# Joao-M-Silva/padel_analytics

Measured on NVIDIA H100. Metric: frames/sec through trackers.runner (all 4 trackers), higher is better.
Workload: dtype f16 storage, f32 accumulate

## Files before the change

padel_analytics_b200/csrc/conv_common.cuh:

```cuda
#pragma once
#include "internal.h"
#include "ptx.cuh"

namespace pb {

__device__ __forceinline__ void bias_act16(const uint32_t (&r)[16], const float* __restrict__ sbias, int act,
                                           float (&v)[16], const __half* __restrict__ res_first = nullptr) {
#pragma unroll
  for (int q = 0; q < 4; ++q) {
    const float4 b = *reinterpret_cast<const float4*>(sbias + 4 * q);
    v[4 * q + 0] = __uint_as_float(r[4 * q + 0]) + b.x;
    v[4 * q + 1] = __uint_as_float(r[4 * q + 1]) + b.y;
    v[4 * q + 2] = __uint_as_float(r[4 * q + 2]) + b.z;
    v[4 * q + 3] = __uint_as_float(r[4 * q + 3]) + b.w;
  }
  if (res_first != nullptr) {
#pragma unroll
    for (int j = 0; j < 16; ++j) v[j] += __half2float(res_first[j]);
  }
  if (act == PB_ACT_SILU) {
#pragma unroll
    for (int i = 0; i < 16; ++i) v[i] = __fdividef(v[i], 1.f + __expf(-v[i]));
  } else if (act == PB_ACT_RELU) {
#pragma unroll
// ... 101 lines not shown
  } else if (kp.out_mode == PB_OUT_F32_NCHW) {
    float* ob = reinterpret_cast<float*>(kp.out);
    const size_t plane = (size_t)kp.Ho * kp.Wo;
    const size_t base = (size_t)px.n * kp.cout_store * plane + (size_t)px.oh * kp.Wo + px.ow;
#pragma unroll
    for (int j = 0; j < 16; ++j)
      if (ch0 + j < kp.cout_store) ob[base + (size_t)(ch0 + j) * plane] = v[j];
  }
}

__device__ __forceinline__ bool epilogue_fast_ok(const ConvKParams& kp) {
  if ((kp.dbg_flags & 2) != 0 && kp.out2_mode == PB_OUT2_NONE) return false;
  if (kp.head_n != 0 || (kp.res != nullptr && ((kp.res_C | kp.res_coff) & 7) != 0)) return false;
  if ((reinterpret_cast<uintptr_t>(kp.out) & 31) != 0) return false;
  if (kp.out_mode == PB_OUT_F16_NHWC || kp.out_mode == PB_OUT_F16_NHWC_UP2)
    return ((kp.out_C | kp.out_coff) & 15) == 0 && (kp.cout_store & 15) == 0;
  if (kp.out_mode == PB_OUT_F32_NHWC) return ((kp.out_C | kp.out_coff) & 7) == 0;
  return false;
}

__device__ __forceinline__ void silu4(float& a, float& b, float& c, float& d) {
  constexpr float kNegLog2e = -1.4426950408889634f;
  const float da = 1.f + ex2_approx(fminf(a * kNegLog2e, 30.f));
  const float db = 1.f + ex2_approx(fminf(b * kNegLog2e, 30.f));
  const float dc = 1.f + ex2_approx(fminf(c * kNegLog2e, 30.f));
  const float dd = 1.f + ex2_approx(fminf(d * kNegLog2e, 30.f));
  const float pab = da * db, pcd = dc * dd;
  const float r = rcp_approx(pab * pcd);
  const float rab = pcd * r, rcd = pab * r;
  a *= db * rab;
  b *= da * rab;
  c *= dd * rcd;
  d *= dc * rcd;
}

struct EpiOut {
  int mode;
  size_t dx, dy;
  int mode2;
  size_t dx2, dy2;
  bool pool_writer;
};

__device__ __forceinline__ void epi_add_res16(const uint4 (&rv)[2], float (&v)[16]) {
#pragma unroll
  for (int g = 0; g < 2; ++g) {
    const __half2* h2 = reinterpret_cast<const __half2*>(&rv[g]);
#pragma unroll
    for (int j = 0; j < 4; ++j) {
      const float2 f = __half22float2(h2[j]);
      v[8 * g + 2 * j] = __fadd_rn(v[8 * g + 2 * j], f.x);
      v[8 * g + 2 * j + 1] = __fadd_rn(v[8 * g + 2 * j + 1], f.y);
    }
  }
}

__device__ __forceinline__ void epi_compute16(int act, int has_res, bool plain_silu, uint32_t (&r)[16],
                                              const float* __restrict__ sbias, const uint4 (&rv)[2], float (&v)[16]) {
#pragma unroll
  for (int q = 0; q < 4; ++q) {
    const float4 b = *reinterpret_cast<const float4*>(sbias + 4 * q);
    v[4 * q + 0] = __uint_as_float(r[4 * q + 0]) + b.x;
    v[4 * q + 1] = __uint_as_float(r[4 * q + 1]) + b.y;
    v[4 * q + 2] = __uint_as_float(r[4 * q + 2]) + b.z;
    v[4 * q + 3] = __uint_as_float(r[4 * q + 3]) + b.w;
  }
// ... 262 lines not shown
```

padel_analytics_b200/csrc/conv_halo.cu:

```cuda
#include <cstdlib>
#include <mutex>
#include <vector>

#include "conv_halo_kernel.cuh"

namespace pb {


static void halo_finish_config(ConvPlan* plan) {
  const ConvKParams& kp = plan->kp;
  plan->smem_bytes = (size_t)kp.a_stages * kp.a_bytes + (size_t)kp.b_stages * kp.b_bytes + sizeof(HaloSmemTail) + 1024;
  plan->threads = kConvThreads;
  plan->grid = kp.total_tiles < num_sms() ? kp.total_tiles : num_sms();
}

int conv_stem_setup(const pb_conv_desc* d, ConvPlan* plan, EncodeTiledFn encode) {
  PB_CHECK(d->ksize == 3 && d->stride == 2 && d->C == 4 && d->cin == 16 && d->c_in_off == 0,
           "conv(stem): needs ksize 3, stride 2, C = 4, cin = 16");
  PB_CHECK(d->cout_pad <= 128, "conv(stem): cout_pad %d > 128", d->cout_pad);
  ConvKParams& kp = plan->kp;
  const int BN = d->cout_pad;
  const int acc_cols = (BN + 31) / 32 * 32;
  int S = 4;
  while (S > 1 && S * acc_cols > 2 * kConvAccRegs) S >>= 1;
  kp.KB = 16;
  kp.kblocks = 1;
  kp.taps = 3;
  kp.hs_S = S;
  kp.hs_P = 8 * S;
  kp.hs_G = 3;
  kp.hs_ntaps = 3;
  kp.hs_sbo_rows = 3 * 8 * S;
  kp.hs_x0 = 0;
  kp.hs_y0 = 0;
  for (int r = 0; r < 3; ++r) kp.hs_tap_off[r] = r * 8 * S;
  for (int r = 0; r < 3; ++r) kp.hs_tap_desc[r] = (kp.hs_tap_off[r] * 32) >> 4;
  kp.BN = BN;
  kp.n_ntiles = 1;
  kp.halo_bytes = 16u * 3u * (uint32_t)(8 * S) * 32u;
  kp.hs_a_row_bytes = 32u;
  const uint32_t pairs = (uint32_t)(8 * S) + 1;
  const uint32_t pitch = pairs * 16u;
  static const int raw = [] {
    const char* e = getenv("PADEL_B200_STEM_RAW");
    return e ? atoi(e) : 1;
  }();
  if (raw) {
    kp.halo_bytes = 17u * 2u * pitch;
    kp.hs_a_row_bytes = 16u;
    kp.hs_sbo_rows = (int)(2u * pitch / 16u);
    for (int r = 0; r < 3; ++r) kp.hs_tap_desc[r] = (int)(((uint32_t)r * pitch) >> 4);
  }
  kp.a_bytes = (kp.halo_bytes + 1023u) & ~1023u;
  kp.b_tx_bytes = 3u * (uint32_t)BN * 32u;
  kp.b_bytes = (kp.b_tx_bytes + 1023u) & ~1023u;
  kp.a_stages = 4;
  kp.b_stages = 1;
  kp.b_resident = 1;
  kp.tiles_w = (kp.Wo + 8 * S - 1) / (8 * S);
  kp.tiles_h = (kp.Ho + 15) / 16;
  kp.tiles_n = kp.N;
  kp.total_tiles = kp.tiles_w * kp.tiles_h * kp.tiles_n;
  halo_finish_config(plan);
  plan->variant = 1;
  {
    const cuuint64_t Wp = (cuuint64_t)d->W + 2, Hp = (cuuint64_t)d->H + 2;
    cuuint64_t dims[5] = {16, (cuuint64_t)d->W / 2, 3, (cuuint64_t)d->H / 2, (cuuint64_t)d->N};
    cuuint64_t strides[4] = {16, Wp * 8, 2 * Wp * 8, Hp * Wp * 8};
    cuuint32_t box[5] = {16, (cuuint32_t)(8 * S), 3, 16, 1};
    cuuint32_t estr[5] = {1, 1, 1, 1, 1};
    CUtensorMapSwizzle swz = CU_TENSOR_MAP_SWIZZLE_32B;
    if (raw) {
      dims[0] = 8, dims[1] = Wp / 2, dims[2] = 2, dims[3] = Hp / 2;
      strides[0] = 16, strides[1] = Wp * 8, strides[2] = 2 * Wp * 8;
      box[0] = 8, box[1] = pairs, box[2] = 2, box[3] = 17;
      swz = CU_TENSOR_MAP_SWIZZLE_NONE;
    }
    CUresult r = encode(&plan->tmap_a, CU_TENSOR_MAP_DATA_TYPE_FLOAT16, 5, const_cast<void*>(d->in), dims, strides,
                        box, estr, CU_TENSOR_MAP_INTERLEAVE_NONE, swz, CU_TENSOR_MAP_L2_PROMOTION_L2_128B,
                        CU_TENSOR_MAP_FLOAT_OOB_FILL_NONE);
    PB_CHECK(r == CUDA_SUCCESS, "conv(stem): cuTensorMapEncodeTiled(A, overlapping rows) failed with %d", (int)r);
  }
  {
    cuuint64_t dims[3] = {16, (cuuint64_t)d->cout_pad, 3};
    cuuint64_t strides[2] = {32, (cuuint64_t)d->cout_pad * 32};
    cuuint32_t box[3] = {16, (cuuint32_t)BN, 3};
    cuuint32_t estr[3] = {1, 1, 1};
    CUresult r = encode(&plan->tmap_w, CU_TENSOR_MAP_DATA_TYPE_FLOAT16, 3, const_cast<void*>(d->weight), dims,
                        strides, box, estr, CU_TENSOR_MAP_INTERLEAVE_NONE, CU_TENSOR_MAP_SWIZZLE_32B,
                        CU_TENSOR_MAP_L2_PROMOTION_L2_256B, CU_TENSOR_MAP_FLOAT_OOB_FILL_NONE);
    PB_CHECK(r == CUDA_SUCCESS, "conv(stem): cuTensorMapEncodeTiled(W) failed with %d", (int)r);
  }
  return 0;
}

int conv_halo_setup(const pb_conv_desc* d, ConvPlan* plan, EncodeTiledFn encode) {
  if (d->ksize != 3 || d->stride != 1 || d->cout_pad > 256) return -1;
  ConvKParams& kp = plan->kp;
  const int BN = d->cout_pad;
  const uint32_t row_bytes = (uint32_t)kp.KB * 2u;
  const int acc_cols = (BN + 31) / 32 * 32;
  const size_t budget = 196 * 1024;
  const uint32_t tap_bytes = (uint32_t)BN * row_bytes;
  const uint32_t res_box = (9u * tap_bytes + 1023u) & ~1023u;
  const size_t res_total = (size_t)kp.kblocks * res_box;
  bool resident = false;
  {
    const char* er = getenv("PADEL_B200_CONV_BRES");
    resident = (!er || atoi(er) != 0) && kp.kblocks <= kHaloMaxB && res_total <= 120 * 1024;
  }
  int bestS = 0, best_cols = 0, G = 1;
  for (int pass = resident ? 0 : 1; pass < 2 && bestS == 0; ++pass) {
    resident = resident && pass == 0;
    for (int S = 4; S >= 1; S >>= 1) {
      if (S * acc_cols > 2 * kConvAccRegs) continue;
      const uint32_t halo = 18u * (uint32_t)(8 * S + 2) * row_bytes;
      const uint32_t a_alloc = (halo + 1023u) & ~1023u;
      int g_fit = 0;
      if (resident) {
        if ((size_t)2 * a_alloc + res_total <= budget) g_fit = 9;
      } else {
        for (int g = 9; g >= 1; g = (g == 9 ? 3 : (g == 3 ? 1 : 0))) {
          const uint32_t ba = ((uint32_t)g * tap_bytes + 1023u) & ~1023u;
          const int min_b = g == 9 ? 2 : (g == 3 ? 3 : 4);
          if ((size_t)2 * a_alloc + (size_t)min_b * ba <= budget) {
            g_fit = g;
            break;
          }
        }
      }
      if (!g_fit) continue;
      const int cols = (d->W + 8 * S - 1) / (8 * S) * 8 * S;
      if (bestS == 0 || (!resident && cols < best_cols)) {
        bestS = S;
        best_cols = cols;
// ... 17 lines not shown
      kp.hs_tap_off[r * 3 + q] = r * P + q;
      kp.hs_tap_desc[r * 3 + q] = (int)(((uint32_t)(r * P + q) * row_bytes) >> 4);
    }
  kp.BN = BN;
  kp.n_ntiles = 1;
  kp.halo_bytes = 18u * (uint32_t)P * row_bytes;
  kp.hs_a_row_bytes = row_bytes;
  kp.a_bytes = (kp.halo_bytes + 1023u) & ~1023u;
  kp.b_tx_bytes = (uint32_t)G * tap_bytes;
  kp.b_bytes = b_alloc;
  kp.a_stages = 2;
  if (resident) {
    kp.b_stages = kp.kblocks;
    int as = (int)((budget - res_total) / kp.a_bytes);
    if (as > kHaloMaxA) as = kHaloMaxA;
    if (as > 2 * kp.kblocks + 1) as = 2 * kp.kblocks + 1;
    kp.a_stages = as < 2 ? 2 : as;
  } else {
    size_t rest = budget - (size_t)2 * kp.a_bytes;
    if (kp.kblocks > 2 && rest > (size_t)kp.a_bytes + 4 * (size_t)b_alloc) {
      kp.a_stages = 3;
      rest -= kp.a_bytes;
    }
    int bs = (int)(rest / b_alloc);
    if (bs > kHaloMaxB) bs = kHaloMaxB;
    if (bs > 9 * kp.kblocks / G * 2) bs = 9 * kp.kblocks / G * 2;
    if (bs < 2) bs = 2;
    kp.b_stages = bs;
  }
  kp.tiles_w = (kp.Wo + 8 * S - 1) / (8 * S);
  kp.tiles_h = (kp.Ho + 15) / 16;
  kp.tiles_n = kp.N;
  kp.total_tiles = kp.tiles_w * kp.tiles_h * kp.tiles_n;
  halo_finish_config(plan);
  plan->variant = 1;

  const CUtensorMapSwizzle swz = kp.KB == 64   ? CU_TENSOR_MAP_SWIZZLE_128B
                                 : kp.KB == 32 ? CU_TENSOR_MAP_SWIZZLE_64B
                                               : CU_TENSOR_MAP_SWIZZLE_32B;
  {
    const cuuint64_t C = (cuuint64_t)d->C, W = (cuuint64_t)d->W, H = (cuuint64_t)d->H;
    cuuint64_t dims[5] = {C, W, 1, H, (cuuint64_t)d->N};
    cuuint64_t strides[4] = {C * 2, W * C * 2, W * C * 2, H * W * C * 2};
    cuuint32_t box[5] = {(cuuint32_t)kp.KB, (cuuint32_t)P, 1, 18, 1};
    cuuint32_t estr[5] = {1, 1, 1, 1, 1};
    CUresult r = encode(&plan->tmap_a, CU_TENSOR_MAP_DATA_TYPE_FLOAT16, 5, const_cast<void*>(d->in), dims, strides,
                        box, estr, CU_TENSOR_MAP_INTERLEAVE_NONE, swz, CU_TENSOR_MAP_L2_PROMOTION_L2_128B,
                        CU_TENSOR_MAP_FLOAT_OOB_FILL_NONE);
    PB_CHECK(r == CUDA_SUCCESS, "conv(halo): cuTensorMapEncodeTiled(A) failed with %d", (int)r);
  }
  {
    cuuint64_t dims[3] = {(cuuint64_t)d->cin, (cuuint64_t)d->cout_pad, 9};
    cuuint64_t strides[2] = {(cuuint64_t)d->cin * 2, (cuuint64_t)d->cin * d->cout_pad * 2};
    cuuint32_t box[3] = {(cuuint32_t)kp.KB, (cuuint32_t)BN, (cuuint32_t)G};
    cuuint32_t estr[3] = {1, 1, 1};
    CUresult r = encode(&plan->tmap_w, CU_TENSOR_MAP_DATA_TYPE_FLOAT16, 3, const_cast<void*>(d->weight), dims,
                        strides, box, estr, CU_TENSOR_MAP_INTERLEAVE_NONE, swz, CU_TENSOR_MAP_L2_PROMOTION_L2_256B,
                        CU_TENSOR_MAP_FLOAT_OOB_FILL_NONE);
    PB_CHECK(r == CUDA_SUCCESS, "conv(halo): cuTensorMapEncodeTiled(W) failed with %d", (int)r);
  }
  return 0;
}

int conv_halo_1x1_setup(const pb_conv_desc* d, ConvPlan* plan, EncodeTiledFn encode) {
  static const int enabled = [] {
    const char* e = getenv("PADEL_B200_CONV_HALO1");
    return e ? atoi(e) : 1;
  }();
  if (!enabled || d->ksize != 1 || d->stride != 1 || d->cout_pad > 256 || d->head_n != 0) return -1;
  if (enabled == 1 && d->cin > 32) return -1;
  if (d->out_mode != PB_OUT_F16_NHWC && d->out_mode != PB_OUT_F16_NHWC_UP2) return -1;
  ConvKParams& kp = plan->kp;
  const int BN = d->cout_pad;
  const uint32_t row_bytes = (uint32_t)kp.KB * 2u;
  const int acc_cols = (BN + 31) / 32 * 32;
  const size_t budget = 196 * 1024;
  const uint32_t tap_bytes = (uint32_t)BN * row_bytes;
  const uint32_t res_box = (tap_bytes + 1023u) & ~1023u;
  const size_t res_total = (size_t)kp.kblocks * res_box;
  if (kp.kblocks > kHaloMaxB || res_total > 120 * 1024) return -1;
  int S = 0;
  for (int s = 4; s >= 1; s >>= 1) {
    if (s * acc_cols > 2 * kConvAccRegs) continue;
    const uint32_t a_alloc = (16u * (uint32_t)(8 * s) * row_bytes + 1023u) & ~1023u;
    if ((size_t)2 * a_alloc + res_total > budget) continue;
    if (s > 1 && d->W <= 8 * (s / 2)) continue;
    S = s;
    break;
  }
  if (S == 0) return -1;
  const int P = 8 * S;
  kp.b_resident = 1;
  kp.hs_S = S;
  kp.hs_P = P;
  kp.hs_G = 1;
  kp.hs_ntaps = 1;
  kp.hs_sbo_rows = P;
  kp.hs_x0 = 0;
  kp.hs_y0 = 0;
  kp.hs_tap_off[0] = 0;
  kp.hs_tap_desc[0] = 0;
  kp.BN = BN;
  kp.n_ntiles = 1;
  kp.halo_bytes = 16u * (uint32_t)P * row_bytes;
  kp.hs_a_row_bytes = row_bytes;
  kp.a_bytes = (kp.halo_bytes + 1023u) & ~1023u;
  kp.b_tx_bytes = tap_bytes;
  kp.b_bytes = res_box;
  kp.b_stages = kp.kblocks;
  {
    int as = (int)((budget - res_total) / kp.a_bytes);
    if (as > kHaloMaxA) as = kHaloMaxA;
    if (as > 2 * kp.kblocks + 1) as = 2 * kp.kblocks + 1;
    kp.a_stages = as < 2 ? 2 : as;
  }
  kp.tiles_w = (kp.Wo + 8 * S - 1) / (8 * S);
  kp.tiles_h = (kp.Ho + 15) / 16;
  kp.tiles_n = kp.N;
  kp.total_tiles = kp.tiles_w * kp.tiles_h * kp.tiles_n;
  halo_finish_config(plan);
  plan->variant = 1;
  const CUtensorMapSwizzle swz = kp.KB == 64   ? CU_TENSOR_MAP_SWIZZLE_128B
                                 : kp.KB == 32 ? CU_TENSOR_MAP_SWIZZLE_64B
                                               : CU_TENSOR_MAP_SWIZZLE_32B;
  {
    const cuuint64_t C = (cuuint64_t)d->C, W = (cuuint64_t)d->W, H = (cuuint64_t)d->H;
    cuuint64_t dims[5] = {C, W, 1, H, (cuuint64_t)d->N};
    cuuint64_t strides[4] = {C * 2, W * C * 2, W * C * 2, H * W * C * 2};
    cuuint32_t box[5] = {(cuuint32_t)kp.KB, (cuuint32_t)P, 1, 16, 1};
    cuuint32_t estr[5] = {1, 1, 1, 1, 1};
    CUresult r = encode(&plan->tmap_a, CU_TENSOR_MAP_DATA_TYPE_FLOAT16, 5, const_cast<void*>(d->in), dims, strides,
                        box, estr, CU_TENSOR_MAP_INTERLEAVE_NONE, swz, CU_TENSOR_MAP_L2_PROMOTION_L2_128B,
                        CU_TENSOR_MAP_FLOAT_OOB_FILL_NONE);
    PB_CHECK(r == CUDA_SUCCESS, "conv(halo 1x1): cuTensorMapEncodeTiled(A) failed with %d", (int)r);
  }
  {
    cuuint64_t dims[3] = {(cuuint64_t)d->cin, (cuuint64_t)d->cout_pad, 1};
    cuuint64_t strides[2] = {(cuuint64_t)d->cin * 2, (cuuint64_t)d->cin * d->cout_pad * 2};
    cuuint32_t box[3] = {(cuuint32_t)kp.KB, (cuuint32_t)BN, 1};
    cuuint32_t estr[3] = {1, 1, 1};
    CUresult r = encode(&plan->tmap_w, CU_TENSOR_MAP_DATA_TYPE_FLOAT16, 3, const_cast<void*>(d->weight), dims,
                        strides, box, estr, CU_TENSOR_MAP_INTERLEAVE_NONE, swz, CU_TENSOR_MAP_L2_PROMOTION_L2_256B,
                        CU_TENSOR_MAP_FLOAT_OOB_FILL_NONE);
    PB_CHECK(r == CUDA_SUCCESS, "conv(halo 1x1): cuTensorMapEncodeTiled(W) failed with %d", (int)r);
  }
  return 0;
}

int conv_halo_s2_setup(const pb_conv_desc* d, ConvPlan* plan, EncodeTiledFn encode) {
  if (d->ksize != 3 || d->stride != 2 || d->cout_pad > 256 || d->c_in_off != 0 || d->C != d->cin ||
      (d->cin != 16 && d->cin != 32))
    return -1;
  ConvKParams& kp = plan->kp;
  const int BN = d->cout_pad;
  const uint32_t row_bytes = (uint32_t)d->cin * 2u;
  const uint32_t a_row = 2u * row_bytes;
  const int acc_cols = (BN + 31) / 32 * 32;
  const uint32_t tap_bytes = (uint32_t)BN * row_bytes;
  const uint32_t b_alloc = (9u * tap_bytes + 1023u) & ~1023u;
  const size_t budget = 196 * 1024;
  int S = 0;
  for (int s = 4; s >= 1; s >>= 1) {
    if (s * acc_cols > 2 * kConvAccRegs) continue;
    const uint32_t halo = 34u * (uint32_t)(8 * s + 1) * a_row;
    if ((size_t)2 * ((halo + 1023u) & ~1023u) + (size_t)2 * b_alloc <= budget) {
      S = s;
      break;
    }
  }
  if (S == 0) return -1;
  const int P = 8 * S + 1;
  kp.KB = d->cin;
  kp.kblocks = 1;
  kp.hs_S = S;
  kp.hs_P = P;
  kp.hs_G = 9;
  kp.hs_ntaps = 9;
  kp.hs_sbo_rows = 2 * P;
  kp.hs_x0 = -1;
  kp.hs_y0 = -1;
  kp.hs_a_row_bytes = a_row;
  for (int r = 0; r < 3; ++r)
    for (int q = 0; q < 3; ++q) {
      const int row = ((r == 0 ? 0 : 1) * 2 + (r == 1 ? 0 : 1)) * P + (q == 0 ? 0 : 1);
      const int half = q == 1 ? 0 : 1;
      kp.hs_tap_off[r * 3 + q] = row;
      kp.hs_tap_desc[r * 3 + q] = (int)(((uint32_t)row * a_row + (uint32_t)half * row_bytes) >> 4);
    }
  kp.BN = BN;
  kp.n_ntiles = 1;
  kp.halo_bytes = 34u * (uint32_t)P * a_row;
  kp.a_bytes = (kp.halo_bytes + 1023u) & ~1023u;
  kp.b_tx_bytes = 9u * tap_bytes;
  kp.b_bytes = b_alloc;
  kp.a_stages = 2;
  kp.b_stages = 1;
  kp.b_resident = 1;
  kp.tiles_w = (kp.Wo + 8 * S - 1) / (8 * S);
  kp.tiles_h = (kp.Ho + 15) / 16;
  kp.tiles_n = kp.N;
  kp.total_tiles = kp.tiles_w * kp.tiles_h * kp.tiles_n;
  halo_finish_config(plan);
  plan->variant = 1;
  {
    const cuuint64_t C = (cuuint64_t)d->C, W = (cuuint64_t)d->W, H = (cuuint64_t)d->H;
    cuuint64_t dims[5] = {2 * C, W / 2, 2, H / 2, (cuuint64_t)d->N};
    cuuint64_t strides[4] = {2 * C * 2, W * C * 2, 2 * W * C * 2, H * W * C * 2};
    cuuint32_t box[5] = {(cuuint32_t)(2 * d->C), (cuuint32_t)P, 2, 17, 1};
    cuuint32_t estr[5] = {1, 1, 1, 1, 1};
    CUresult r = encode(&plan->tmap_a, CU_TENSOR_MAP_DATA_TYPE_FLOAT16, 5, const_cast<void*>(d->in), dims, strides,
                        box, estr, CU_TENSOR_MAP_INTERLEAVE_NONE,
                        a_row == 128 ? CU_TENSOR_MAP_SWIZZLE_128B : CU_TENSOR_MAP_SWIZZLE_64B,
                        CU_TENSOR_MAP_L2_PROMOTION_L2_128B, CU_TENSOR_MAP_FLOAT_OOB_FILL_NONE);
    PB_CHECK(r == CUDA_SUCCESS, "conv(halo s2): cuTensorMapEncodeTiled(A) failed with %d", (int)r);
  }
  {
    cuuint64_t dims[3] = {(cuuint64_t)d->cin, (cuuint64_t)d->cout_pad, 9};
    cuuint64_t strides[2] = {(cuuint64_t)d->cin * 2, (cuuint64_t)d->cin * d->cout_pad * 2};
    cuuint32_t box[3] = {(cuuint32_t)d->cin, (cuuint32_t)BN, 9};
    cuuint32_t estr[3] = {1, 1, 1};
    CUresult r = encode(&plan->tmap_w, CU_TENSOR_MAP_DATA_TYPE_FLOAT16, 3, const_cast<void*>(d->weight), dims,
                        strides, box, estr, CU_TENSOR_MAP_INTERLEAVE_NONE,
                        row_bytes == 64 ? CU_TENSOR_MAP_SWIZZLE_64B : CU_TENSOR_MAP_SWIZZLE_32B,
                        CU_TENSOR_MAP_L2_PROMOTION_L2_256B, CU_TENSOR_MAP_FLOAT_OOB_FILL_NONE);
    PB_CHECK(r == CUDA_SUCCESS, "conv(halo s2): cuTensorMapEncodeTiled(W) failed with %d", (int)r);
  }
  return 0;
}

static HaloKernelFn halo_kernel_pick(const ConvPlan* plan) {
  const ConvKParams& kp = plan->kp;
  const int S = kp.hs_S, steps = kp.KB / 16, BN = kp.BN;
  if (plan->epi == PB_EPI_SILU) return halo_kernel_lookup<PB_EPI_SILU>(S, steps, BN);
  if (plan->epi == PB_EPI_RELU) return halo_kernel_lookup<PB_EPI_RELU>(S, steps, BN);
  if (plan->epi == PB_EPI_SILU_RES) return halo_kernel_lookup<PB_EPI_SILU_RES>(S, steps, BN);
  return halo_kernel_lookup<PB_EPI_GENERIC>(S, steps, BN);
}

int conv_halo_launch(const ConvPlan* plan, cudaStream_t stream) {
  const ConvKParams& kp = plan->kp;
  HaloKernelFn fn = halo_kernel_pick(plan);
  PB_CHECK(fn != nullptr, "conv(halo): no kernel instantiation for S=%d, k-steps=%d, N=%d, epilogue class %d",
           kp.hs_S, kp.KB / 16, kp.BN, plan->epi);
  PB_CUDA((cudaError_t)ensure_dynamic_smem(reinterpret_cast<const void*>(fn), 227 * 1024));
  cudaError_t le = launch_ex(fn, dim3(plan->grid), dim3(plan->threads), plan->smem_bytes, stream, 1, plan->pdl != 0,
                             plan->tmap_a, plan->tmap_w, plan->kp);
  PB_CHECK(le == cudaSuccess, "conv(halo): launch failed: %s (grid %d, threads %d, smem %zu, tiles %d, S %d, BN %d, KB %d)",
           cudaGetErrorString(le), plan->grid, plan->threads, plan->smem_bytes, kp.total_tiles, kp.hs_S, kp.BN, kp.KB);
  count_launch();
  return 0;
}

}
```

padel_analytics_b200/csrc/conv_halo_kernel.cuh:

```cuda
#pragma once
#include "conv_common.cuh"
#include "internal.h"
#include "ptx.cuh"

namespace pb {

constexpr int kHaloMaxA = 4;
constexpr int kHaloMaxB = 12;

struct HaloSmemTail {
  uint64_t a_full[kHaloMaxA];
  uint64_t a_empty[kHaloMaxA];
  uint64_t b_full[kHaloMaxB];
  uint64_t b_empty[kHaloMaxB];
  float bias[kConvMaxCout];
  float scratch[kConvConsumerWarps * kEpiScratchFloats];
};

struct HaloTile {
  int tw, th, n;
};
__device__ __forceinline__ HaloTile halo_decode(const ConvKParams& kp, int tile) {
  HaloTile t;
  int q;
  fast_divmod(q, t.tw, tile, kp.fd_w);
  fast_divmod(t.n, t.th, q, kp.fd_h);
  return t;
}

template <int kS, int kSteps, int kBN, int kEpi>
__global__ void __launch_bounds__(kConvThreads, 1)
conv_halo_kernel(const __grid_constant__ CUtensorMap tmap_a, const __grid_constant__ CUtensorMap tmap_w,
                 const __grid_constant__ ConvKParams kp) {
  constexpr int kNch = (kBN + 31) / 32;
  constexpr int kAcc = kS * kNch * 16;
  static_assert(kAcc <= kConvAccRegs, "accumulators of kS sub-tiles must fit the registers");
  extern __shared__ __align__(1024) uint8_t smem_raw[];
  uint8_t* smem = smem_raw + ((1024u - (smem_u32(smem_raw) & 1023u)) & 1023u);
  uint8_t* a_base = smem;
  uint8_t* b_base = smem + (size_t)kp.a_stages * kp.a_bytes;
  HaloSmemTail* tail = reinterpret_cast<HaloSmemTail*>(b_base + (size_t)kp.b_stages * kp.b_bytes);

  const int warp = threadIdx.x >> 5;
  const int lane = threadIdx.x & 31;
  constexpr int S = kS;
  const int G = kp.hs_G;
  const uint32_t row_bytes = (uint32_t)kp.KB * 2u;
  const uint32_t a_row_bytes = kp.hs_a_row_bytes;
  const int tap_groups = kp.hs_ntaps / G;

  if (warp == 0 && lane == 0) {
    tma_prefetch_desc(&tmap_a);
    for (int i = 0; i < kp.a_stages; ++i) {
      mbar_init(&tail->a_full[i], 1);
      mbar_init(&tail->a_empty[i], kConvConsumerWarps);
    }
    for (int i = 0; i < kp.b_stages; ++i) {
      mbar_init(&tail->b_full[i], 1);
      mbar_init(&tail->b_empty[i], kConvConsumerWarps);
    }
    fence_mbar_init();
  }
  if (warp == 1 && lane == 0) tma_prefetch_desc(&tmap_w);
  for (int i = threadIdx.x; i < kp.cout_pad; i += blockDim.x) tail->bias[i] = kp.bias[i];
  __syncthreads();
  griddep_launch_dependents();
  if (warp != 1) griddep_wait();

  if (warp < 4) {
    warpgroup_reg_dealloc<kConvProducerRegs>();
    if (warp == 0 && lane == 0) {
      int st = 0;
      uint32_t ph = 0;
      for (int tile = blockIdx.x; tile < kp.total_tiles; tile += gridDim.x) {
        const HaloTile t = halo_decode(kp, tile);
        for (int cb = 0; cb < kp.kblocks; ++cb) {
          mbar_wait(&tail->a_empty[st], ph ^ 1);
          mbar_arrive_expect_tx(&tail->a_full[st], kp.halo_bytes);
          tma_load_5d(a_base + (size_t)st * kp.a_bytes, &tmap_a, &tail->a_full[st], kp.c_in_off + cb * kp.KB,
                      t.tw * 8 * S + kp.hs_x0, 0, t.th * 16 + kp.hs_y0, t.n);
          if (++st == kp.a_stages) {
            st = 0;
            ph ^= 1;
          }
        }
      }
    } else if (warp == 1 && lane == 0) {
      int st = 0;
      uint32_t ph = 0;
      for (int tile = blockIdx.x; tile < kp.total_tiles; tile += gridDim.x) {
        for (int cb = 0; cb < kp.kblocks; ++cb) {
          for (int tg = 0; tg < tap_groups; ++tg) {
            if (!kp.b_resident) mbar_wait(&tail->b_empty[st], ph ^ 1);
            mbar_arrive_expect_tx(&tail->b_full[st], kp.b_tx_bytes);
            tma_load_3d(b_base + (size_t)st * kp.b_bytes, &tmap_w, &tail->b_full[st], cb * kp.KB, 0, tg * G);
            if (++st == kp.b_stages) {
// ... 30 lines not shown
      const uint64_t a_desc0 = wgmma_desc(smem_u32(a_base + (size_t)ast * kp.a_bytes), a_row_bytes, sbo) + g_units;
      for (int tg = 0; tg < tap_groups; ++tg) {
        mbar_wait(&tail->b_full[bst], kp.b_resident ? 0u : bph);
        const uint64_t b_desc0 = wgmma_desc_kmajor(smem_u32(b_base + (size_t)bst * kp.b_bytes), row_bytes);
        wgmma_fence();
        for (int ti = 0; ti < G; ++ti) {
          const int tap = tg * G + ti;
          mma_n<kBN, kS, kSteps>(acc, a_desc0 + (uint64_t)(uint32_t)kp.hs_tap_desc[tap], sub_units,
                                 b_desc0 + (uint64_t)((uint32_t)ti * tap_b_units), (uint32_t)((cb | tap) != 0));
        }
        wgmma_commit();
        if (prev_b >= 0) {
          wgmma_wait<1>();
          if (!kp.b_resident) consumer_release(&tail->b_empty[prev_b], lane);
          if (prev_a >= 0) consumer_release(&tail->a_empty[prev_a], lane);
          prev_a = -1;
        }
        prev_b = bst;
        if (++bst == kp.b_stages) {
          bst = 0;
          bph ^= 1;
        }
      }
      prev_a = ast;
      if (++ast == kp.a_stages) {
        ast = 0;
        aph ^= 1;
      }
    }
    wgmma_wait<0>();
    wgmma_fence_operands(acc);
    if (!kp.b_resident) consumer_release(&tail->b_empty[prev_b], lane);
    consumer_release(&tail->a_empty[prev_a], lane);
    const int oh = t.th * 16 + row, ow0 = t.tw * 8 * S + col;
    epilogue_tile<kEpi, kS, kNch>(kp, acc, S, 0, tail->bias, scr, lane, [&](int j, bool& pool_writer) {
      EpiPix px;
      px.n = t.n;
      px.oh = oh;
      px.ow = ow0 + 8 * j;
      px.valid = (px.ow < kp.Wo) && (px.oh < kp.Ho);
      px.pix = ((size_t)px.n * kp.Ho + px.oh) * kp.Wo + px.ow;
      pool_writer = ((row | col) & 1) == 0;
      return px;
    });
  }
}

typedef void (*HaloKernelFn)(CUtensorMap, CUtensorMap, ConvKParams);

template <int kS, int kSteps, int kEpi>
static HaloKernelFn halo_kernel_for_bn(int BN) {
  switch (BN) {
#define PB_HALO_BN(n_)                                                                     \
  case n_:                                                                                 \
    if constexpr (kS * ((n_ + 31) / 32) * 16 <= kConvAccRegs) return conv_halo_kernel<kS, kSteps, n_, kEpi>; \
    break;
    PB_HALO_BN(16) PB_HALO_BN(32) PB_HALO_BN(48) PB_HALO_BN(64) PB_HALO_BN(80) PB_HALO_BN(96) PB_HALO_BN(112)
    PB_HALO_BN(128) PB_HALO_BN(144) PB_HALO_BN(160) PB_HALO_BN(176) PB_HALO_BN(192) PB_HALO_BN(208)
    PB_HALO_BN(224) PB_HALO_BN(240) PB_HALO_BN(256)
#undef PB_HALO_BN
    default: break;
  }
  return nullptr;
}

template <int kEpi>
HaloKernelFn halo_kernel_lookup(int S, int steps, int BN) {
#define PB_HALO_CASE(s_, k_) \
  if (S == s_ && steps == k_) return halo_kernel_for_bn<s_, k_, kEpi>(BN);
  PB_HALO_CASE(1, 1) PB_HALO_CASE(1, 2) PB_HALO_CASE(1, 4)
  PB_HALO_CASE(2, 1) PB_HALO_CASE(2, 2) PB_HALO_CASE(2, 4)
  PB_HALO_CASE(4, 1) PB_HALO_CASE(4, 2) PB_HALO_CASE(4, 4)
#undef PB_HALO_CASE
  return nullptr;
}


extern template HaloKernelFn halo_kernel_lookup<PB_EPI_GENERIC>(int, int, int);
extern template HaloKernelFn halo_kernel_lookup<PB_EPI_SILU>(int, int, int);
extern template HaloKernelFn halo_kernel_lookup<PB_EPI_RELU>(int, int, int);
extern template HaloKernelFn halo_kernel_lookup<PB_EPI_SILU_RES>(int, int, int);
// ... 3 lines not shown
```

padel_analytics_b200/csrc/internal.h:

```cpp
#pragma once
#include <cuda.h>
#include <cuda_fp16.h>
#include <cuda_runtime.h>

#include <atomic>
#include <cstdarg>
#include <cstdlib>
#include <cstdio>
#include <string>

#include "../../include/padel_b200.h"

namespace pb {

void set_error(const char* fmt, ...);
extern std::atomic<long long> g_launches;
inline void count_launch(int n = 1) { g_launches.fetch_add(n, std::memory_order_relaxed); }
int num_sms();
int ensure_dynamic_smem(const void* func, size_t bytes);
bool pdl_enabled();
int plan_pdl();

#ifdef __CUDACC__
template <typename... KArgs, typename... Args>
// ... 76 lines not shown
}
#endif

struct ConvKParams {
  int N, Ho, Wo;
  int tiles_w, tiles_h, tiles_n, n_ntiles, total_tiles;
  FastDiv fd_w, fd_h, fd_nt;
  int tw_log2, th_log2;
  int taps, kblocks, KB, BN, stages, cout_pad;
  int c_in_off;
  int tap_dc[9], tap_dw[9], tap_d2[9], tap_dh[9];
  const float* bias;
  int act;
  const __half* res;
  int res_C, res_coff;
  int res_first;
  void* out;
  int out_C, out_coff, out_mode, cout_store;
  void* out2;
  int out2_C, out2_coff, out2_mode;
  uint32_t a_bytes, b_bytes, b_tx_bytes;
  const float* head_w;
  const float* head_b;
  int head_n;
  float* head_out;
  int b_resident;
  int hs_S, hs_P, hs_G, a_stages, b_stages;
  uint32_t halo_bytes;
  uint32_t hs_a_row_bytes;
  int hs_ntaps, hs_sbo_rows, hs_x0, hs_y0, hs_tile_h;
  int hs_tap_off[9];
  int hs_tap_desc[9];
  int dbg_flags;
};

struct ConvPlan {
  pb_conv_desc desc;
  ConvKParams kp;
  CUtensorMap tmap_a;
  CUtensorMap tmap_w;
  int grid;
  int threads;
  size_t smem_bytes;
  int variant;
  int pdl;
  int epi;
};

#define PB_EPI_GENERIC 0
#define PB_EPI_SILU 1
#define PB_EPI_RELU 2
#define PB_EPI_SILU_RES 3
#define PB_EPI_F32 4
int conv_epi_class(const pb_conv_desc* d, const ConvKParams& kp);

typedef CUresult (*EncodeTiledFn)(CUtensorMap*, CUtensorMapDataType, cuuint32_t, void*, const cuuint64_t*,
                                  const cuuint64_t*, const cuuint32_t*, const cuuint32_t*, CUtensorMapInterleave,
                                  CUtensorMapSwizzle, CUtensorMapL2promotion, CUtensorMapFloatOOBfill);
int conv_halo_setup(const pb_conv_desc* d, ConvPlan* plan, EncodeTiledFn encode);
int conv_stem_setup(const pb_conv_desc* d, ConvPlan* plan, EncodeTiledFn encode);
int conv_halo_s2_setup(const pb_conv_desc* d, ConvPlan* plan, EncodeTiledFn encode);
int conv_halo_1x1_setup(const pb_conv_desc* d, ConvPlan* plan, EncodeTiledFn encode);
int conv_halo_launch(const ConvPlan* plan, cudaStream_t stream);
int conv_plan_build(const pb_conv_desc* d, ConvPlan* plan);
int conv_plan_launch(const ConvPlan* plan, cudaStream_t stream);
int conv_reference_launch(const pb_conv_desc* d, cudaStream_t stream);

int launch_maxpool2(const void* in, int N, int H, int W, int C, int c_off, int c, void* out, int out_C,
                    int out_coff, cudaStream_t s);
int launch_upsample2(const void* in, int N, int H, int W, int C, int c_off, int c, void* out, int out_C,
                     int out_coff, cudaStream_t s);
int launch_sppf_pool(void* buf, int N, int H, int W, int C, int c, cudaStream_t s);
int launch_pointwise_head(const void* in, int N, int H, int W, int C, const float* w, const float* b, int n_out,
// ... 4 lines not shown
```

padel_analytics_b200/csrc/ptx.cuh:

```cuda
#pragma once
#include <cstdint>
#include <cuda.h>
#include <cuda_fp16.h>
#include <cuda_runtime.h>

namespace pb {

__device__ __forceinline__ uint32_t smem_u32(const void* p) {
  return static_cast<uint32_t>(__cvta_generic_to_shared(p));
}

__device__ __forceinline__ void mbar_init(uint64_t* bar, uint32_t count) {
  asm volatile("mbarrier.init.shared::cta.b64 [%0], %1;" ::"r"(smem_u32(bar)), "r"(count));
}
__device__ __forceinline__ void fence_mbar_init() {
  asm volatile("fence.mbarrier_init.release.cluster;" ::: "memory");
}
__device__ __forceinline__ void fence_proxy_async_smem() {
  asm volatile("fence.proxy.async.shared::cta;" ::: "memory");
}
__device__ __forceinline__ void mbar_arrive_expect_tx(uint64_t* bar, uint32_t bytes) {
  asm volatile("mbarrier.arrive.expect_tx.shared::cta.b64 _, [%0], %1;" ::"r"(smem_u32(bar)), "r"(bytes)
               : "memory");
}
// ... 14 lines not shown
__device__ __forceinline__ void mbar_wait(uint64_t* bar, uint32_t parity) {
  while (!mbar_try_wait(bar, parity)) {
  }
}

__device__ __forceinline__ unsigned long long globaltimer_ns() {
  unsigned long long t;
  asm volatile("mov.u64 %0, %%globaltimer;" : "=l"(t));
  return t;
}
__device__ __forceinline__ void griddep_wait() { asm volatile("griddepcontrol.wait;" ::: "memory"); }
__device__ __forceinline__ void griddep_launch_dependents() {
  asm volatile("griddepcontrol.launch_dependents;" ::: "memory");
}

__device__ __forceinline__ void tma_prefetch_desc(const CUtensorMap* m) {
  asm volatile("prefetch.tensormap [%0];" ::"l"(reinterpret_cast<uint64_t>(m)) : "memory");
}
__device__ __forceinline__ void tma_load_3d(void* dst, const CUtensorMap* m, uint64_t* bar, int c0, int c1,
                                            int c2) {
  asm volatile(
      "cp.async.bulk.tensor.3d.shared::cluster.global.mbarrier::complete_tx::bytes [%0], [%1, {%3, %4, %5}], "
      "[%2];" ::"r"(smem_u32(dst)),
      "l"(reinterpret_cast<uint64_t>(m)), "r"(smem_u32(bar)), "r"(c0), "r"(c1), "r"(c2)
      : "memory");
}
__device__ __forceinline__ void tma_load_5d(void* dst, const CUtensorMap* m, uint64_t* bar, int c0, int c1,
                                            int c2, int c3, int c4) {
  asm volatile(
      "cp.async.bulk.tensor.5d.shared::cluster.global.mbarrier::complete_tx::bytes [%0], [%1, {%3, %4, %5, %6, "
      "%7}], [%2];" ::"r"(smem_u32(dst)),
      "l"(reinterpret_cast<uint64_t>(m)), "r"(smem_u32(bar)), "r"(c0), "r"(c1), "r"(c2), "r"(c3), "r"(c4)
      : "memory");
}

template <int kRegs>
__device__ __forceinline__ void warpgroup_reg_dealloc() {
  asm volatile("setmaxnreg.dec.sync.aligned.u32 %0;" ::"n"(kRegs));
}
template <int kRegs>
__device__ __forceinline__ void warpgroup_reg_alloc() {
  asm volatile("setmaxnreg.inc.sync.aligned.u32 %0;" ::"n"(kRegs));
}

__device__ __forceinline__ float ex2_approx(float x) {
  float y;
  asm("ex2.approx.ftz.f32 %0, %1;" : "=f"(y) : "f"(x));
  return y;
}
__device__ __forceinline__ float rcp_approx(float x) {
  float y;
  asm("rcp.approx.ftz.f32 %0, %1;" : "=f"(y) : "f"(x));
  return y;
}

__device__ __forceinline__ void wgmma_fence() { asm volatile("wgmma.fence.sync.aligned;" ::: "memory"); }
__device__ __forceinline__ void wgmma_commit() { asm volatile("wgmma.commit_group.sync.aligned;" ::: "memory"); }
template <int kPending>
__device__ __forceinline__ void wgmma_wait() {
  asm volatile("wgmma.wait_group.sync.aligned %0;" ::"n"(kPending) : "memory");
}
template <int kN>
__device__ __forceinline__ void wgmma_fence_operands(float (&d)[kN]) {
#pragma unroll
  for (int i = 0; i < kN; ++i) asm volatile("" : "+f"(d[i])::"memory");
}
// ... 91 lines not shown
```

Baseline: 1246.

## Add TMA-store epilogue for halo conv kernels via stmatrix staging

Adds an epilogue path for the halo conv kernels. Each consumer warpgroup applies bias and activation, packs the results to f16 with stmatrix into a swizzled shared-memory staging buffer, and issues TMA bulk tensor stores, including the upsample and fused 2x2 maxpool outputs. This replaces per-thread global stores so output writes are coalesced and asynchronous. The staging buffer takes shared memory, so the planner may cut A/B pipeline stages, and new named-barrier syncs are added. It also adds a SiLU variant that shares the reciprocal between lane pairs via a shuffle.

```diff
diff --git a/padel_analytics_b200/csrc/conv_common.cuh b/padel_analytics_b200/csrc/conv_common.cuh
--- a/padel_analytics_b200/csrc/conv_common.cuh
+++ b/padel_analytics_b200/csrc/conv_common.cuh
@@ -157,6 +157,18 @@
   b *= da * rab;
   c *= dd * rcd;
   d *= dc * rcd;
+}
+
+__device__ __forceinline__ void silu2_frag(float& a, float& b) {
+  constexpr float kNegLog2e = -1.4426950408889634f;
+  const float da = 1.f + ex2_approx(fminf(a * kNegLog2e, 30.f));
+  const float db = 1.f + ex2_approx(fminf(b * kNegLog2e, 30.f));
+  const float p = da * db;
+  const float po = __shfl_xor_sync(0xffffffffu, p, 1);
+  const float r = rcp_approx(p * po);
+  const float rp = po * r;
+  a *= db * rp;
+  b *= da * rp;
 }
 
 struct EpiOut {
diff --git a/padel_analytics_b200/csrc/conv_halo.cu b/padel_analytics_b200/csrc/conv_halo.cu
--- a/padel_analytics_b200/csrc/conv_halo.cu
+++ b/padel_analytics_b200/csrc/conv_halo.cu
@@ -7,9 +7,73 @@
 namespace pb {
 
 
+constexpr size_t kHaloSmemBudget = 196 * 1024;
+
+static int halo_plan_store(const pb_conv_desc* d, ConvPlan* plan, EncodeTiledFn encode) {
+  const size_t budget = kHaloSmemBudget;
+  static const int enabled = [] {
+    const char* e = getenv("PADEL_B200_CONV_TMA_STORE");
+    return e ? atoi(e) : 1;
+  }();
+  ConvKParams& kp = plan->kp;
+  kp.st_bytes = 0;
+  kp.st_maps = 0;
+  kp.st_pool = 0;
+  const bool f16 = d->out_mode == PB_OUT_F16_NHWC || d->out_mode == PB_OUT_F16_NHWC_UP2;
+  if (!enabled || kp.dbg_flags != 0 || d->res || d->head_n != 0 || !f16 || plan->epi == PB_EPI_SILU_RES ||
+      d->cout_store != kp.BN || ((d->out_C | d->out_coff) & 7) != 0)
+    return 0;
+  if (!kp.b_resident && kp.kblocks > 2) return 0;
+  const uint32_t st = (uint32_t)kp.hs_S * (uint32_t)kp.BN * 256u;
+  int as = kp.a_stages, bs = kp.b_stages;
+  auto total = [&] { return (size_t)as * kp.a_bytes + (size_t)bs * kp.b_bytes + st; };
+  while (total() > budget) {
+    if (!kp.b_resident && bs > 4) --bs;
+    else if (as > 2) --as;
+    else if (!kp.b_resident && bs > 3) --bs;
+    else return 0;
+  }
+  const int S = kp.hs_S, bc = halo_store_box_channels(kp.BN);
+  const CUtensorMapSwizzle swz = bc == 64 ? CU_TENSOR_MAP_SWIZZLE_128B
+                                 : bc == 32 ? CU_TENSOR_MAP_SWIZZLE_64B
+                                            : CU_TENSOR_MAP_SWIZZLE_32B;
+  int nm = 0;
+  auto add = [&](void* out, int C, int coff, int W, int H, int up, int dy, int dx, int bw, int bh) {
+    const size_t pxb = (size_t)C * 2;
+    char* base = reinterpret_cast<char*>(out) + ((size_t)(dy * up * W + dx) * C + coff) * 2;
+    cuuint64_t dims[4] = {(cuuint64_t)kp.BN, (cuuint64_t)W, (cuuint64_t)H, (cuuint64_t)kp.N};
+    cuuint64_t strides[3] = {up * pxb, (cuuint64_t)up * up * W * pxb, (cuuint64_t)up * up * W * H * pxb};
+    cuuint32_t box[4] = {(cuuint32_t)bc, (cuuint32_t)bw, (cuuint32_t)bh, 1};
+    cuuint32_t estr[4] = {1, 1, 1, 1};
+    return encode(&plan->tmap_o.m[nm++], CU_TENSOR_MAP_DATA_TYPE_FLOAT16, 4, base, dims, strides, box, estr,
+                  CU_TENSOR_MAP_INTERLEAVE_NONE, swz, CU_TENSOR_MAP_L2_PROMOTION_NONE, CU_TENSOR_MAP_FLOAT_OOB_FILL_NONE);
+  };
+  CUresult r = CUDA_SUCCESS;
+  const int up = d->out_mode == PB_OUT_F16_NHWC_UP2 ? 2 : 1;
+  for (int dy = 0; dy < up; ++dy)
+    for (int dx = 0; dx < up; ++dx)
+      if (r == CUDA_SUCCESS) r = add(d->out, d->out_C, d->out_coff, kp.Wo, kp.Ho, up, dy, dx, 8 * S, 8);
+  if (d->out2_mode == PB_OUT2_UP2) {
+    for (int dy = 0; dy < 2; ++dy)
+      for (int dx = 0; dx < 2; ++dx)
+        if (r == CUDA_SUCCESS) r = add(d->out2, d->out2_C, d->out2_coff, kp.Wo, kp.Ho, 2, dy, dx, 8 * S, 8);
+  }
+  kp.st_maps = nm;
+  if (d->out2_mode == PB_OUT2_POOL2 && r == CUDA_SUCCESS) {
+    r = add(d->out2, d->out2_C, d->out2_coff, kp.Wo / 2, kp.Ho / 2, 1, 0, 0, 4 * S, 4);
+    kp.st_pool = 1;
+  }
+  PB_CHECK(r == CUDA_SUCCESS, "conv(halo): cuTensorMapEncodeTiled(store) failed with %d", (int)r);
+  kp.st_bytes = st;
+  kp.a_stages = as;
+  kp.b_stages = bs;
+  return 0;
+}
+
 static void halo_finish_config(ConvPlan* plan) {
   const ConvKParams& kp = plan->kp;
-  plan->smem_bytes = (size_t)kp.a_stages * kp.a_bytes + (size_t)kp.b_stages * kp.b_bytes + sizeof(HaloSmemTail) + 1024;
+  plan->smem_bytes = (size_t)kp.a_stages * kp.a_bytes + (size_t)kp.b_stages * kp.b_bytes + kp.st_bytes +
+                     sizeof(HaloSmemTail) + 1024;
   plan->threads = kConvThreads;
   plan->grid = kp.total_tiles < num_sms() ? kp.total_tiles : num_sms();
 }
@@ -61,6 +125,7 @@
   kp.tiles_h = (kp.Ho + 15) / 16;
   kp.tiles_n = kp.N;
   kp.total_tiles = kp.tiles_w * kp.tiles_h * kp.tiles_n;
+  if (halo_plan_store(d, plan, encode) != 0) return 1;
   halo_finish_config(plan);
   plan->variant = 1;
   {
@@ -100,7 +165,7 @@
   const int BN = d->cout_pad;
   const uint32_t row_bytes = (uint32_t)kp.KB * 2u;
   const int acc_cols = (BN + 31) / 32 * 32;
-  const size_t budget = 196 * 1024;
+  const size_t budget = kHaloSmemBudget;
   const uint32_t tap_bytes = (uint32_t)BN * row_bytes;
   const uint32_t res_box = (9u * tap_bytes + 1023u) & ~1023u;
   const size_t res_total = (size_t)kp.kblocks * res_box;
@@ -184,6 +249,7 @@
   kp.tiles_h = (kp.Ho + 15) / 16;
   kp.tiles_n = kp.N;
   kp.total_tiles = kp.tiles_w * kp.tiles_h * kp.tiles_n;
+  if (halo_plan_store(d, plan, encode) != 0) return 1;
   halo_finish_config(plan);
   plan->variant = 1;
 
@@ -226,7 +292,7 @@
   const int BN = d->cout_pad;
   const uint32_t row_bytes = (uint32_t)kp.KB * 2u;
   const int acc_cols = (BN + 31) / 32 * 32;
-  const size_t budget = 196 * 1024;
+  const size_t budget = kHaloSmemBudget;
   const uint32_t tap_bytes = (uint32_t)BN * row_bytes;
   const uint32_t res_box = (tap_bytes + 1023u) & ~1023u;
   const size_t res_total = (size_t)kp.kblocks * res_box;
@@ -270,6 +336,7 @@
   kp.tiles_h = (kp.Ho + 15) / 16;
   kp.tiles_n = kp.N;
   kp.total_tiles = kp.tiles_w * kp.tiles_h * kp.tiles_n;
+  if (halo_plan_store(d, plan, encode) != 0) return 1;
   halo_finish_config(plan);
   plan->variant = 1;
   const CUtensorMapSwizzle swz = kp.KB == 64   ? CU_TENSOR_MAP_SWIZZLE_128B
@@ -310,7 +377,7 @@
   const int acc_cols = (BN + 31) / 32 * 32;
   const uint32_t tap_bytes = (uint32_t)BN * row_bytes;
   const uint32_t b_alloc = (9u * tap_bytes + 1023u) & ~1023u;
-  const size_t budget = 196 * 1024;
+  const size_t budget = kHaloSmemBudget;
   int S = 0;
   for (int s = 4; s >= 1; s >>= 1) {
     if (s * acc_cols > 2 * kConvAccRegs) continue;
@@ -352,6 +419,7 @@
   kp.tiles_h = (kp.Ho + 15) / 16;
   kp.tiles_n = kp.N;
   kp.total_tiles = kp.tiles_w * kp.tiles_h * kp.tiles_n;
+  if (halo_plan_store(d, plan, encode) != 0) return 1;
   halo_finish_config(plan);
   plan->variant = 1;
   {
@@ -391,14 +459,19 @@
 
 int conv_halo_launch(const ConvPlan* plan, cudaStream_t stream) {
   const ConvKParams& kp = plan->kp;
+  const int tma_store = kp.st_bytes != 0;
   HaloKernelFn fn = halo_kernel_pick(plan);
-  PB_CHECK(fn != nullptr, "conv(halo): no kernel instantiation for S=%d, k-steps=%d, N=%d, epilogue class %d",
-           kp.hs_S, kp.KB / 16, kp.BN, plan->epi);
+  PB_CHECK(fn != nullptr,
+           "conv(halo): no kernel instantiation for S=%d, k-steps=%d, N=%d, epilogue class %d (TMA store %d)", kp.hs_S,
+           kp.KB / 16, kp.BN, plan->epi, tma_store);
   PB_CUDA((cudaError_t)ensure_dynamic_smem(reinterpret_cast<const void*>(fn), 227 * 1024));
   cudaError_t le = launch_ex(fn, dim3(plan->grid), dim3(plan->threads), plan->smem_bytes, stream, 1, plan->pdl != 0,
-                             plan->tmap_a, plan->tmap_w, plan->kp);
-  PB_CHECK(le == cudaSuccess, "conv(halo): launch failed: %s (grid %d, threads %d, smem %zu, tiles %d, S %d, BN %d, KB %d)",
-           cudaGetErrorString(le), plan->grid, plan->threads, plan->smem_bytes, kp.total_tiles, kp.hs_S, kp.BN, kp.KB);
+                             plan->tmap_a, plan->tmap_w, plan->kp, plan->tmap_o);
+  PB_CHECK(le == cudaSuccess,
+           "conv(halo): launch failed: %s (grid %d, threads %d, smem %zu, tiles %d, S %d, k-steps %d, N %d, epilogue "
+           "class %d, TMA store %d)",
+           cudaGetErrorString(le), plan->grid, plan->threads, plan->smem_bytes, kp.total_tiles, kp.hs_S, kp.KB / 16,
+           kp.BN, plan->epi, tma_store);
   count_launch();
   return 0;
 }
diff --git a/padel_analytics_b200/csrc/conv_halo_kernel.cuh b/padel_analytics_b200/csrc/conv_halo_kernel.cuh
--- a/padel_analytics_b200/csrc/conv_halo_kernel.cuh
+++ b/padel_analytics_b200/csrc/conv_halo_kernel.cuh
@@ -28,10 +28,126 @@
   return t;
 }
 
+__host__ __device__ constexpr int halo_store_box_channels(int bn) { return bn % 64 == 0 ? 64 : (bn % 32 == 0 ? 32 : 16); }
+
+template <int kEpi, int kS, int kBN, int kAcc>
+__device__ __forceinline__ void halo_epilogue_tma(const ConvKParams& kp, const HaloStoreMaps& maps,
+                                                  const float (&acc)[kAcc], const float* __restrict__ sbias,
+                                                  uint8_t* stage, const HaloTile& t, int g, int wq, int lane) {
+  constexpr int kAS = (kBN + 31) / 32 * 16;
+  constexpr int kBC = halo_store_box_channels(kBN);
+  constexpr uint32_t kRow = 2u * kBC;
+  constexpr uint32_t kBox = 64u * kS * kRow;
+  constexpr uint32_t kPoolBox = 16u * kS * kRow;
+  constexpr int kCpr = kBC / 8;
+  const int act = kEpi == PB_EPI_SILU ? PB_ACT_SILU : (kEpi == PB_EPI_RELU ? PB_ACT_RELU : kp.act);
+  const bool pool = kp.st_pool != 0;
+  const bool leader = (threadIdx.x & 127) == 0;
+  const int bar = 1 + g;
+  const int q = lane & 3, mi = lane >> 3;
+  const uint32_t sbase = smem_u32(stage);
+  const uint32_t key = (((uint32_t)(lane & 7) * kRow) >> 7) & (uint32_t)(kCpr - 1);
+  const uint32_t lane_row = sbase + (uint32_t)((2 * wq + (mi & 1)) * 8 * kS + (lane & 7)) * kRow;
+  const uint32_t hi = (uint32_t)(mi >> 1);
+
+  if (leader) bulk_wait_group_read0();
+  named_barrier_sync(bar, 128);
+#pragma unroll
+  for (int j = 0; j < kS; ++j) {
+#pragma unroll
+    for (int i = 0; i < kBN / 8; i += 2) {
+      uint32_t h[4];
+#pragma unroll
+      for (int u = 0; u < 2; ++u) {
+        const float* a4 = acc + j * kAS + 4 * (i + u);
+        const float2 b = *reinterpret_cast<const float2*>(sbias + 8 * (i + u) + 2 * q);
+        float v0 = a4[0] + b.x, v1 = a4[1] + b.y, v2 = a4[2] + b.x, v3 = a4[3] + b.y;
+        if (act == PB_ACT_SILU) {
+          silu2_frag(v0, v1);
+          silu2_frag(v2, v3);
+        } else if (act == PB_ACT_RELU) {
+          v0 = fmaxf(v0, 0.f);
+          v1 = fmaxf(v1, 0.f);
+          v2 = fmaxf(v2, 0.f);
+          v3 = fmaxf(v3, 0.f);
+        } else if (act == PB_ACT_SIGMOID) {
+          v0 = __fdividef(1.f, 1.f + __expf(-v0));
+          v1 = __fdividef(1.f, 1.f + __expf(-v1));
+          v2 = __fdividef(1.f, 1.f + __expf(-v2));
+          v3 = __fdividef(1.f, 1.f + __expf(-v3));
+        }
+        const __half2 top = __floats2half2_rn(v0, v1), bot = __floats2half2_rn(v2, v3);
+        h[2 * u] = *reinterpret_cast<const uint32_t*>(&top);
+        h[2 * u + 1] = *reinterpret_cast<const uint32_t*>(&bot);
+      }
+      const uint32_t chunk = ((uint32_t)(i % kCpr) + hi) ^ key;
+      stmatrix_x4(lane_row + (uint32_t)(i / kCpr) * kBox + (uint32_t)(8 * j) * kRow + (chunk << 4), h[0], h[1], h[2],
+                  h[3]);
+    }
+  }
+  fence_proxy_async_smem();
+  named_barrier_sync(bar, 128);
+  const int x0 = t.tw * 8 * kS, y0 = t.th * 16 + 8 * g;
+  if (leader) {
+    for (int m = 0; m < kp.st_maps; ++m)
+#pragma unroll
+      for (int b = 0; b < kBN / kBC; ++b) tma_store_4d(&maps.m[m], stage + b * kBox, b * kBC, x0, y0, t.n);
+    bulk_commit_group();
+  }
+  if (pool) {
+    constexpr int kUnits = 2 * kS * kBN, kPer = (kUnits + 127) / 128;
+    auto addr = [&](int pix, int cc, uint32_t box) {
+      const uint32_t k = (((uint32_t)pix * kRow) >> 7) & (uint32_t)(kCpr - 1);
+      return sbase + (uint32_t)(cc / kCpr) * box + (uint32_t)pix * kRow + ((((uint32_t)(cc % kCpr)) ^ k) << 4);
+    };
+    const int tid = threadIdx.x & 127;
+    uint4 pv[kPer];
+#pragma unroll
+    for (int k = 0; k < kPer; ++k) {
+      const int un = tid + 128 * k, cc = un % (kBN / 8), pp = un / (kBN / 8);
+      const int src = (pp / (4 * kS)) * 16 * kS + 2 * (pp % (4 * kS));
+      if (un < kUnits) {
+        uint4 w[4];
+#pragma unroll
+        for (int e = 0; e < 4; ++e)
+          asm volatile("ld.shared.v4.b32 {%0, %1, %2, %3}, [%4];"
+                       : "=r"(w[e].x), "=r"(w[e].y), "=r"(w[e].z), "=r"(w[e].w)
+                       : "r"(addr(src + (e >> 1) * 8 * kS + (e & 1), cc, kBox))
+                       : "memory");
+        const __half2* h0 = reinterpret_cast<const __half2*>(&w[0]);
+        const __half2* h1 = reinterpret_cast<const __half2*>(&w[1]);
+        const __half2* h2 = reinterpret_cast<const __half2*>(&w[2]);
+        const __half2* h3 = reinterpret_cast<const __half2*>(&w[3]);
+        __half2* o = reinterpret_cast<__half2*>(&pv[k]);
+#pragma unroll
+        for (int c = 0; c < 4; ++c) o[c] = __hmax2(__hmax2(h0[c], h1[c]), __hmax2(h2[c], h3[c]));
+      }
+    }
+    if (leader) bulk_wait_group_read0();
+    named_barrier_sync(bar, 128);
+#pragma unroll
+    for (int k = 0; k < kPer; ++k) {
+      const int un = tid + 128 * k;
+      if (un < kUnits)
+        asm volatile("st.shared.v4.b32 [%0], {%1, %2, %3, %4};" ::"r"(addr(un / (kBN / 8), un % (kBN / 8), kPoolBox)),
+                     "r"(pv[k].x), "r"(pv[k].y), "r"(pv[k].z), "r"(pv[k].w)
+                     : "memory");
+    }
+    fence_proxy_async_smem();
+    named_barrier_sync(bar, 128);
+    if (leader) {
+#pragma unroll
+      for (int b = 0; b < kBN / kBC; ++b)
+        tma_store_4d(&maps.m[kp.st_maps], stage + b * kPoolBox, b * kBC, x0 >> 1, y0 >> 1, t.n);
+      bulk_commit_group();
+    }
+  }
+}
+
 template <int kS, int kSteps, int kBN, int kEpi>
 __global__ void __launch_bounds__(kConvThreads, 1)
 conv_halo_kernel(const __grid_constant__ CUtensorMap tmap_a, const __grid_constant__ CUtensorMap tmap_w,
-                 const __grid_constant__ ConvKParams kp) {
+                 const __grid_constant__ ConvKParams kp, const __grid_constant__ HaloStoreMaps tmap_o) {
   constexpr int kNch = (kBN + 31) / 32;
   constexpr int kAcc = kS * kNch * 16;
   static_assert(kAcc <= kConvAccRegs, "accumulators of kS sub-tiles must fit the registers");
@@ -39,7 +155,8 @@
   uint8_t* smem = smem_raw + ((1024u - (smem_u32(smem_raw) & 1023u)) & 1023u);
   uint8_t* a_base = smem;
   uint8_t* b_base = smem + (size_t)kp.a_stages * kp.a_bytes;
-  HaloSmemTail* tail = reinterpret_cast<HaloSmemTail*>(b_base + (size_t)kp.b_stages * kp.b_bytes);
+  uint8_t* st_base = b_base + (size_t)kp.b_stages * kp.b_bytes;
+  HaloSmemTail* tail = reinterpret_cast<HaloSmemTail*>(st_base + kp.st_bytes);
 
   const int warp = threadIdx.x >> 5;
   const int lane = threadIdx.x & 31;
@@ -62,6 +179,7 @@
     fence_mbar_init();
   }
   if (warp == 1 && lane == 0) tma_prefetch_desc(&tmap_w);
+  if (warp == 2 && lane < kp.st_maps + kp.st_pool) tma_prefetch_desc(&tmap_o.m[lane]);
   for (int i = threadIdx.x; i < kp.cout_pad; i += blockDim.x) tail->bias[i] = kp.bias[i];
   __syncthreads();
   griddep_launch_dependents();
@@ -158,6 +276,13 @@
     wgmma_fence_operands(acc);
     if (!kp.b_resident) consumer_release(&tail->b_empty[prev_b], lane);
     consumer_release(&tail->a_empty[prev_a], lane);
+    if constexpr (kEpi != PB_EPI_SILU_RES) {
+      if (kp.st_bytes != 0) {
+        halo_epilogue_tma<kEpi, kS, kBN>(kp, tmap_o, acc, tail->bias, st_base + (size_t)g * (kp.st_bytes / 2), t, g,
+                                         wq, lane);
+        continue;
+      }
+    }
     const int oh = t.th * 16 + row, ow0 = t.tw * 8 * S + col;
     epilogue_tile<kEpi, kS, kNch>(kp, acc, S, 0, tail->bias, scr, lane, [&](int j, bool& pool_writer) {
       EpiPix px;
@@ -170,9 +295,10 @@
       return px;
     });
   }
-}
-
-typedef void (*HaloKernelFn)(CUtensorMap, CUtensorMap, ConvKParams);
+  if (kp.st_bytes != 0 && (threadIdx.x & 127) == 0) bulk_wait_group0();
+}
+
+typedef void (*HaloKernelFn)(CUtensorMap, CUtensorMap, ConvKParams, HaloStoreMaps);
 
 template <int kS, int kSteps, int kEpi>
 static HaloKernelFn halo_kernel_for_bn(int BN) {
diff --git a/padel_analytics_b200/csrc/internal.h b/padel_analytics_b200/csrc/internal.h
--- a/padel_analytics_b200/csrc/internal.h
+++ b/padel_analytics_b200/csrc/internal.h
@@ -132,6 +132,13 @@
   int hs_tap_off[9];
   int hs_tap_desc[9];
   int dbg_flags;
+  uint32_t st_bytes;
+  int st_maps, st_pool;
+};
+
+constexpr int kHaloStoreMaps = 5;
+struct HaloStoreMaps {
+  CUtensorMap m[kHaloStoreMaps];
 };
 
 struct ConvPlan {
@@ -139,6 +146,7 @@
   ConvKParams kp;
   CUtensorMap tmap_a;
   CUtensorMap tmap_w;
+  HaloStoreMaps tmap_o;
   int grid;
   int threads;
   size_t smem_bytes;
diff --git a/padel_analytics_b200/csrc/ptx.cuh b/padel_analytics_b200/csrc/ptx.cuh
--- a/padel_analytics_b200/csrc/ptx.cuh
+++ b/padel_analytics_b200/csrc/ptx.cuh
@@ -70,6 +70,28 @@
       "%7}], [%2];" ::"r"(smem_u32(dst)),
       "l"(reinterpret_cast<uint64_t>(m)), "r"(smem_u32(bar)), "r"(c0), "r"(c1), "r"(c2), "r"(c3), "r"(c4)
       : "memory");
+}
+
+__device__ __forceinline__ void tma_store_4d(const CUtensorMap* m, const void* src, int c0, int c1, int c2, int c3) {
+  asm volatile("cp.async.bulk.tensor.4d.global.shared::cta.bulk_group [%0, {%2, %3, %4, %5}], [%1];" ::"l"(
+                   reinterpret_cast<uint64_t>(m)),
+               "r"(smem_u32(src)), "r"(c0), "r"(c1), "r"(c2), "r"(c3)
+               : "memory");
+}
+__device__ __forceinline__ void bulk_commit_group() { asm volatile("cp.async.bulk.commit_group;" ::: "memory"); }
+__device__ __forceinline__ void bulk_wait_group_read0() {
+  asm volatile("cp.async.bulk.wait_group.read 0;" ::: "memory");
+}
+__device__ __forceinline__ void bulk_wait_group0() { asm volatile("cp.async.bulk.wait_group 0;" ::: "memory"); }
+
+__device__ __forceinline__ void named_barrier_sync(int id, int count) {
+  asm volatile("bar.sync %0, %1;" ::"r"(id), "r"(count) : "memory");
+}
+
+__device__ __forceinline__ void stmatrix_x4(uint32_t addr, uint32_t r0, uint32_t r1, uint32_t r2, uint32_t r3) {
+  asm volatile("stmatrix.sync.aligned.m8n8.x4.shared.b16 [%0], {%1, %2, %3, %4};" ::"r"(addr), "r"(r0), "r"(r1),
+               "r"(r2), "r"(r3)
+               : "memory");
 }
 
 template <int kRegs>
```

Result: faster. 1307 (median of 6 runs) (+4.9%).
